# mandt-lab/shallow-ntc

Measured on AMD Instinct MI355X. Metric: decode Mpixels/s + (bpp, PSNR) on Kodak, two_layer_syn, higher is better.
Workload: dtype f32

## Files before the change

include/sntc.h:

```cpp
#ifndef SNTC_H_
#define SNTC_H_

#include <stddef.h>
#include <stdint.h>

#ifdef __cplusplus
extern "C" {
#endif

#define SNTC_VERSION 100

enum {
  SNTC_OK = 0,
  SNTC_ERR_BAD_SHAPE = 1,
  SNTC_ERR_UNSUPPORTED = 2,
  SNTC_ERR_HIP = 3,
  SNTC_ERR_NONFINITE = 4,
  SNTC_ERR_NO_DEVICE = 5
};

const char* sntc_last_error(void);
int sntc_version(void);
int sntc_device_count(void);
int sntc_device_arch(int device, char* buf, size_t buflen);
// ... 113 lines not shown
int sntc_conv_launch_order(const sntc_conv_plan* plan, int n, int h, int w, int* column_major);
int64_t sntc_conv_tune_workspace_bytes(const sntc_conv_plan* plan, int n, int h, int w);
int sntc_conv_plan_tune(sntc_conv_plan* plan, const float* x, int n, int h, int w, float* y, const float* res,
                        const float* aux, void* workspace, size_t workspace_bytes, int reps, int* variant, int* stream_k,
                        void* stream);
int sntc_conv_plan_candidates(const sntc_conv_plan* plan, int n, int h, int w, int* variants, int* stream_k, int capacity);
int sntc_conv_plan_set_choice(sntc_conv_plan* plan, int n, int h, int w, int variant, int stream_k);
int sntc_conv_plan_clear_tuning(sntc_conv_plan* plan);
int sntc_conv_plan_drop_choice(sntc_conv_plan* plan, int n, int h, int w, int ncols);

int sntc_conv_columns_supported(const sntc_conv_plan* plan, int ncols);
int sntc_conv_forward_columns(const sntc_conv_plan* plan, const float* x, int n, int h, int w, float* y, const float* res,
                              const float* aux, void* workspace, size_t workspace_bytes, void* stream, int ncols);
int64_t sntc_conv_columns_flops(const sntc_conv_plan* plan, int n, int h, int w, int ncols);
int64_t sntc_conv_columns_workspace_bytes(const sntc_conv_plan* plan, int n, int h, int w, int ncols);
int sntc_conv_columns_launch_info(const sntc_conv_plan* plan, int n, int h, int w, int ncols, int* variant, int* nblocks,
                                  int* column_major);
int64_t sntc_conv_columns_tune_workspace_bytes(const sntc_conv_plan* plan, int n, int h, int w, int ncols);
int sntc_conv_columns_tune(sntc_conv_plan* plan, const float* x, int n, int h, int w, int ncols, float* y, void* workspace,
                           size_t workspace_bytes, int reps, int* variant, int* stream_k, void* stream);
int sntc_conv_columns_candidates(const sntc_conv_plan* plan, int n, int h, int w, int ncols, int* variants, int* stream_k,
                                 int capacity);
int sntc_conv_columns_set_choice(sntc_conv_plan* plan, int n, int h, int w, int ncols, int variant, int stream_k);

int sntc_gdn_small(const float* x, int64_t npix, int c, const float* beta, const float* gamma,
                   int inverse, int alpha, int epsilon_is_half, float* y, void* stream);

int sntc_two_layer_tail(const float* t, int n, int hh, int wh, int ch, int has_res, int act_kind,
                        const float* beta, const float* gamma, const float* w2, const float* b2,
                        int k2, int s2, int cout, float* x_hat, void* stream);
int sntc_two_layer_tail_pixels(const float* t, int n, int hh, int wh, int ch, int has_res, int act_kind,
                               const float* beta, const float* gamma, const float* w2, const float* b2, int k2, int s2,
                               int cout, int h, int w, const float* ref, uint8_t* pixels, uint64_t* sse, void* stream);

int sntc_pad_reflect(const float* x, int n, int h, int w, int c, int hp, int wp, float* y, void* stream);
int sntc_pad_zero(const float* x, int n, int h, int w, int c, int top, int left, int hp, int wp, float* y, void* stream);
int sntc_crop(const float* x, int n, int hp, int wp, int c, int h, int w, float* y, void* stream);
int sntc_depth_to_space(const float* x, int n, int h, int w, int c, int block, float* y, void* stream);
int sntc_concat_channels(const float* a, int ca, const float* b, int cb, int64_t npix, float* y, void* stream);
int sntc_pixels_sse(const float* x, const float* x_hat, int n, int h, int w, int c, int hs, int ws,
                    uint8_t* pixels_out, unsigned long long* sse_out, void* stream);
int sntc_block_sse(const float* x, const uint8_t* pixels, int n, int h, int w, int c, int block, uint32_t* out, void* stream);
int sntc_float_sse(const float* x, const float* x_hat, int n, int h, int w, int c, int hs, int ws,
                   double* sse_out, void* stream);

typedef struct sntc_prior sntc_prior;
int sntc_prior_create(int channels, int nlayers, const int* widths, const float* matrices,
                      const float* biases, const float* factors, void* stream, sntc_prior** prior);
void sntc_prior_destroy(sntc_prior* prior);

int sntc_entropy_factorized(const sntc_prior* prior, const float* z, int n, int64_t hw, float* z_hat,
                            double* bits, int values_only, void* stream);

int sntc_entropy_scale_normal(const float* y, const float* hyper, int n, int64_t hw, int c,
                              float* y_hat, int32_t* symbols, double* bits, int values_only,
                              void* stream);
int sntc_dequant_scale_normal(const int32_t* symbols, const float* hyper, int n, int64_t hw, int c,
                              float* y_hat, void* stream);
int sntc_dequant_mean(const int32_t* symbols, const float* mu, int n, int64_t hw, int c, int mu_stride, float* y_hat,
                      void* stream);

int64_t sntc_rans_cap_words(int64_t elems_per_image, int segments);
int sntc_rans_encode(const int32_t* values, const uint16_t* table_ids, int nimages, int64_t elems_per_image, int segments,
                     int lanes, const uint16_t* cdf, const uint32_t* meta, int ntables, int total_entries, int64_t cap_words,
                     uint16_t* scratch, int32_t* len_words, void* stream);
int sntc_rans_compact(const uint16_t* scratch, int64_t cap_words, const int32_t* len_words, const int64_t* offsets,
// ... 133 lines not shown
```

shallow-ntc_amd/_capi.py:

```python
from __future__ import annotations

import ctypes as C
import os
from pathlib import Path

_PKG = Path(__file__).resolve().parent
LIB_PATH = Path(os.environ.get("SNTC_LIB", _PKG / "lib" / "libsntc_hip.so"))

OK, ERR_BAD_SHAPE, ERR_UNSUPPORTED, ERR_HIP, ERR_NONFINITE, ERR_NO_DEVICE = range(6)

CONV2D, CONV2D_TRANSPOSE, SIGNAL_DOWN, SIGNAL_UP = range(4)
ACT_NONE, ACT_RELU, ACT_LEAKY_RELU, ACT_SIGMOID = range(4)
PRO_NONE, PRO_ABS, PRO_SQUARE = range(3)
EPI_STORE, EPI_ADD, EPI_GATE, EPI_RES_DIV, EPI_RES_MUL, EPI_RES_DIV_SQRT, EPI_RES_MUL_SQRT, EPI_MASK_RELU, EPI_MASK_LEAKY = range(9)


class SntcError(RuntimeError):
    def __init__(self, code, msg):
        super().__init__(f"sntc error {code}: {msg}")
        self.code = code


class NonFiniteError(SntcError, ValueError):
    """Mirrors tf.debugging.check_numerics' InvalidArgumentError (reference mshyper/models.py:308-309,356)."""
# ... 126 lines not shown
                                        _P, _P, _P]),
    "sntc_step_map_symbols": (C.c_int, [_P, _P, C.c_int, C.c_int64, C.c_int, C.c_int, _P, _P, _P, _P, _P, _P]),
    "sntc_step_map_table_ids": (C.c_int, [_P, C.c_int, C.c_int64, C.c_int, _P, _P, _P]),
    "sntc_dequant_step_map": (C.c_int, [_P, _P, C.c_int, C.c_int64, C.c_int, C.c_int, _P, _P, _P, _P]),
    "sntc_step_map_ladder_cost": (C.c_int, [_P, _P, C.c_int, C.c_int64, C.c_int, C.c_int, _P, _P, _P, _P, C.c_int, _P, C.c_int,
                                            C.c_int, _P, _P, _P]),
    "sntc_step_ladder_dequant": (C.c_int, [_P, _P, C.c_int, C.c_int64, C.c_int, C.c_int, _P, _P, C.c_int, _P, _P]),
    "sntc_step_map_ladder_dequant": (C.c_int, [_P, _P, C.c_int, C.c_int64, C.c_int, C.c_int, _P, _P, _P, C.c_int, _P, _P]),
    "sntc_ssim_scale": (C.c_int, [_P, _P, C.c_int, C.c_int, C.c_int, C.c_int, C.c_float, _P, _P, _P]),
    "sntc_avgpool2_symmetric": (C.c_int, [_P, C.c_int, C.c_int, C.c_int, C.c_int, _P, _P]),
    "sntc_pixels_float": (C.c_int, [_P, C.c_int, C.c_int, C.c_int, C.c_int, C.c_int, C.c_int, _P, _P]),
    "sntc_msssim_inputs": (C.c_int, [_P, _P, C.c_int, C.c_int, C.c_int, C.c_int, C.c_int, C.c_int, _P, _P, _P, _P]),
    "sntc_msssim_finish": (C.c_int, [_P, C.POINTER(C.c_double), C.POINTER(C.c_double), C.c_int, C.c_int, C.c_int, C.c_double,
                                     _P, _P, _P]),
    "sntc_ssim_scale_grad": (C.c_int, [_P, _P, C.c_int, C.c_int, C.c_int, C.c_int, C.c_float, _P, C.c_int, _P, C.c_int, C.c_int,
                                       C.c_float, _P, _P]),
    "sntc_avgpool2_symmetric_grad": (C.c_int, [_P, C.c_int, C.c_int, C.c_int, C.c_int, _P, _P]),
    "sntc_sga_factorized_fwd": (C.c_int, [_P, _P, C.c_int, C.c_int64, C.c_float, _P, C.c_uint64, C.c_uint64, _P, _P, _P, _P, _P]),
    "sntc_sga_normal_fwd": (C.c_int, [_P, _P, C.c_int, C.c_int64, C.c_int, C.c_float, _P, C.c_uint64, C.c_uint64, _P, _P, _P,
                                      _P, _P, _P]),
    "sntc_sga_normal_bwd": (C.c_int, [_P, _P, _P, _P, C.c_float, C.c_int64, C.c_int, _P, _P, _P]),
    "sntc_sga_normal_step_fwd": (C.c_int, [_P, _P, C.c_int, C.c_int64, C.c_int, C.c_float, _P, C.c_uint64, C.c_uint64, _P, _P, _P,
                                           _P, _P, _P, _P, _P, _P]),
    "sntc_sga_normal_step_bwd": (C.c_int, [_P, _P, _P, _P, C.c_float, C.c_int, C.c_int64, C.c_int, _P, _P, _P, _P, _P, _P]),
    "sntc_uq_sample": (C.c_int, [_P, _P, C.c_int64, C.c_int, C.c_int, C.c_int, C.c_float, _P, C.c_uint64, C.c_uint64, _P, _P]),
    "sntc_sga_chain": (C.c_int, [_P, _P, _P, C.c_float, C.c_int64, _P, _P]),
    "sntc_sga_normal_step_map_fwd": (C.c_int, [_P, _P, C.c_int, C.c_int64, C.c_int, C.c_float, _P, C.c_uint64, C.c_uint64, _P, _P, _P,
                                               _P, _P, _P, _P, _P]),
    "sntc_sga_normal_step_map_bwd": (C.c_int, [_P, _P, _P, _P, C.c_float, C.c_int, C.c_int64, C.c_int, _P, _P, _P, _P, _P]),
    "sntc_distortion_grad_weighted": (C.c_int, [_P, _P, C.c_int, C.c_int, C.c_int, C.c_int, C.c_int, C.c_int, C.c_float, _P, C.c_int,
                                                C.c_int, C.c_int, _P, _P, _P, _P]),
    "sntc_block_sse": (C.c_int, [_P, _P, C.c_int, C.c_int, C.c_int, C.c_int, C.c_int, _P, _P]),
    "sntc_distortion_grad": (C.c_int, [_P, _P, C.c_int, C.c_int, C.c_int, C.c_int, C.c_int, C.c_int, C.c_float, _P, _P, _P]),
    "sntc_two_layer_tail_bwd": (C.c_int, [_P, _P, C.c_int64, C.c_int, C.c_int, C.c_int, _P, _P, C.c_int, _P, _P, _P, _P]),
    "sntc_two_layer_out_adjoint": (C.c_int, [_P, C.c_int, C.c_int, C.c_int, C.c_int, _P, C.c_int, C.c_int, C.c_int, _P, _P]),
    "sntc_adam_step": (C.c_int, [_P, _P, _P, _P, C.c_int64, C.c_float, C.c_float, C.c_float, C.c_float, C.c_int64, C.c_float, _P]),
    "sntc_conv_wgrad_workspace_bytes": (C.c_int64, [C.c_int] * 9),
    "sntc_conv_wgrad": (C.c_int, [C.c_int] * 6 + [_P, _P, C.c_int, C.c_int, C.c_int, _P, C.c_int, _P, C.c_int64, _P]),
    "sntc_bias_grad_workspace_bytes": (C.c_int64, [C.c_int64, C.c_int]),
    "sntc_bias_grad": (C.c_int, [_P, C.c_int64, C.c_int, _P, C.c_int, _P, C.c_int64, _P]),
    "sntc_act_backward": (C.c_int, [_P, _P, C.c_int64, C.c_int, _P, _P]),
    "sntc_gate_forward": (C.c_int, [_P, _P, _P, C.c_int64, _P, _P]),
    "sntc_gate_backward": (C.c_int, [_P, _P, _P, C.c_int64, _P, _P, _P]),
    "sntc_axpy": (C.c_int, [_P, _P, C.c_float, C.c_int64, _P]),
    "sntc_noise_add": (C.c_int, [_P, C.c_int64, _P, C.c_uint64, C.c_uint64, _P, _P]),
    "sntc_sumsq": (C.c_int, [_P, C.c_int64, _P, _P]),
    "sntc_two_layer_hidden": (C.c_int, [_P, C.c_int64, C.c_int, C.c_int, C.c_int, _P, _P, _P, _P]),
    "sntc_gdn_reparam_forward": (C.c_int, [_P, C.c_int64, C.c_float, C.c_float, _P, _P]),
    "sntc_gdn_reparam_backward": (C.c_int, [_P, _P, C.c_int64, C.c_float, _P, _P]),
    "sntc_noisy_normal": (C.c_int, [_P, _P, C.c_int, C.c_int64, C.c_int, _P, _P, _P, _P]),
    "sntc_noisy_factorized": (C.c_int, [_P, _P, C.c_int, C.c_int64, _P, _P, _P, _P]),
    "sntc_gdn_apply": (C.c_int, [_P, _P, C.c_int64, C.c_int, _P, _P]),
    "sntc_gdn_backward_prep": (C.c_int, [_P, _P, _P, C.c_int64, C.c_int, _P, _P, _P]),
    "sntc_gdn_backward_finish": (C.c_int, [_P, _P, _P, _P, C.c_int64, C.c_int, _P, _P]),
    "sntc_small_matmul": (C.c_int, [_P, _P, C.c_int, C.c_int, C.c_int64, C.c_int, _P, _P]),
    "sntc_transpose_last2": (C.c_int, [_P, C.c_int, C.c_int, C.c_int, _P, _P]),
    "sntc_prior_record_floats": (C.c_int, [_P]),
    "sntc_prior_update": (C.c_int, [_P, _P, _P, _P, _P]),
    "sntc_prior_param_grad": (C.c_int, [_P, _P, _P, _P, C.c_float, _P, _P, _P, _P]),
}

_lib = None


def load():
    global _lib
# ... 46 lines not shown
```

shallow-ntc_amd/csrc/pixel.hip:

```cpp
#include <algorithm>
#include "sntc_internal.h"

namespace sntc {

typedef float f32x4 __attribute__((ext_vector_type(4)));

__global__ void pad_reflect_kernel(const float* __restrict__ x, int h, int w, int c, int hp, int wp,
                                   float* __restrict__ y, int64_t total) {
  for (int64_t i = blockIdx.x * (int64_t)blockDim.x + threadIdx.x; i < total; i += (int64_t)gridDim.x * blockDim.x) {
    const int k = (int)(i % c);
    int64_t t = i / c;
    const int j = (int)(t % wp);
    t /= wp;
    const int r = (int)(t % hp);
    const int64_t b = t / hp;
    const int sr = r < h ? r : 2 * h - 2 - r;
    const int sj = j < w ? j : 2 * w - 2 - j;
    y[i] = x[((b * h + sr) * w + sj) * c + k];
  }
}

__global__ void __launch_bounds__(256) pad_zero_kernel(const float* __restrict__ x, int h, int w, int c, int top, int left, int hp, int wp,
                                                       float* __restrict__ y) {
  const int64_t row = blockIdx.y;
  const int64_t b = row / hp;
  const int r = (int)(row - b * hp) - top;
  const bool row_ok = (unsigned)r < (unsigned)h;
  const int lo = left * c, hi = (left + w) * c, len = wp * c;
  const float* src = x + ((b * h + (row_ok ? r : 0)) * (int64_t)w) * c - lo;
  float* dst = y + row * (int64_t)len;
  for (int j = blockIdx.x * blockDim.x + threadIdx.x; j < len; j += gridDim.x * blockDim.x)
    dst[j] = (row_ok && j >= lo && j < hi) ? src[j] : 0.0f;
}

__global__ void crop_kernel(const float* __restrict__ x, int hp, int wp, int c, int h, int w, float* __restrict__ y,
                            int64_t total) {
  for (int64_t i = blockIdx.x * (int64_t)blockDim.x + threadIdx.x; i < total; i += (int64_t)gridDim.x * blockDim.x) {
    const int k = (int)(i % c);
// ... 125 lines not shown
  for (int i = threadIdx.x; i < C * C; i += blockDim.x) sg[i] = gamma[i];
  for (int i = threadIdx.x; i < C; i += blockDim.x) sb[i] = beta[i];
  __syncthreads();
  for (int64_t p = blockIdx.x * (int64_t)blockDim.x + threadIdx.x; p < npix; p += (int64_t)gridDim.x * blockDim.x) {
    float v[C], pool[C];
#pragma unroll
    for (int i = 0; i < C; i += 4) {
      const f32x4 t = *reinterpret_cast<const f32x4*>(x + p * C + i);
      v[i] = t[0]; v[i + 1] = t[1]; v[i + 2] = t[2]; v[i + 3] = t[3];
    }
#pragma unroll
    for (int i = 0; i < C; ++i) pool[i] = alpha == 1 ? fabsf(v[i]) : v[i] * v[i];
#pragma unroll
    for (int j0 = 0; j0 < C; j0 += 4) {
      f32x4 o;
#pragma unroll
      for (int e = 0; e < 4; ++e) {
        const int j = j0 + e;
        float nrm = sb[j];
#pragma unroll
        for (int i = 0; i < C; ++i) nrm += pool[i] * sg[i * C + j];
        if (eps_half) nrm = sqrtf(nrm);
        o[e] = inverse ? v[j] * nrm : v[j] / nrm;
      }
      *reinterpret_cast<f32x4*>(y + p * C + j0) = o;
    }
  }
}

constexpr int tail_px(int ch) { return (ch / 4) % 2 ? ch : ch + 4; }
constexpr int tail_row(int ch) { return (18 * tail_px(ch) + 63) / 64 * 64; }

template <int CH>
__global__ void __launch_bounds__(256) two_layer_tail_kernel(const float* __restrict__ t, int hh, int wh, int has_res,
                                                             int act_kind, const float* __restrict__ beta,
                                                             const float* __restrict__ gamma, const float* __restrict__ w2,
                                                             const float* __restrict__ b2, float* __restrict__ xhat,
                                                             int oh, int ow, const float* __restrict__ ref,
                                                             uint8_t* __restrict__ pix, unsigned long long* __restrict__ sse) {
  constexpr int TQ = 16, TH = TQ + 2;
  constexpr int PX = tail_px(CH), ROW = tail_row(CH);
  extern __shared__ __attribute__((aligned(16))) char smem[];
  float* sh = reinterpret_cast<float*>(smem);
  float* sg = sh + TH * ROW;
  float* sb = sg + CH * CH;
  const int img = blockIdx.z;
  const int qy0 = blockIdx.y * TQ, qx0 = blockIdx.x * TQ;
  const int c2 = has_res ? 2 * CH : CH;
  const bool use_gdn = act_kind == 1 || act_kind == 2;
  if (use_gdn) {
    for (int i = threadIdx.x; i < CH * CH; i += 256) sg[i] = gamma[i];
    for (int i = threadIdx.x; i < CH; i += 256) sb[i] = beta[i];
  }
  __syncthreads();
  for (int p = threadIdx.x; p < TH * TH; p += 256) {
    const int ly = p / TH, lx = p - ly * TH;
    const int iy = qy0 - 2 + ly, ix = qx0 - 2 + lx;
    float* dst = sh + ly * ROW + lx * PX;
    if ((unsigned)iy < (unsigned)hh && (unsigned)ix < (unsigned)wh) {
      const float* src = t + (((int64_t)img * hh + iy) * wh + ix) * c2;
      float v[CH];
#pragma unroll
      for (int i = 0; i < CH; i += 4) {
        const f32x4 q = *reinterpret_cast<const f32x4*>(src + i);
        v[i] = q[0]; v[i + 1] = q[1]; v[i + 2] = q[2]; v[i + 3] = q[3];
      }
#pragma unroll
      for (int j0 = 0; j0 < CH; j0 += 4) {
        f32x4 o;
#pragma unroll
        for (int e = 0; e < 4; ++e) {
          const int j = j0 + e;
          float r = v[j];
          if (use_gdn) {
            float nrm = sb[j];
#pragma unroll
            for (int i = 0; i < CH; ++i) nrm += fabsf(v[i]) * sg[i * CH + j];
            r = act_kind == 1 ? v[j] * nrm : v[j] / nrm;
          } else if (act_kind == 3) {
            r = fmaxf(r, 0.0f);
          } else if (act_kind == 4) {
            r = r >= 0.0f ? r : 0.2f * r;
          }
          o[e] = r;
        }
        if (has_res) {
          const f32x4 q = *reinterpret_cast<const f32x4*>(src + CH + j0);
          o = o + q;
        }
        *reinterpret_cast<f32x4*>(dst + j0) = o;
      }
    } else {
#pragma unroll
      for (int i = 0; i < CH; i += 4) *reinterpret_cast<f32x4*>(dst + i) = f32x4{0.f, 0.f, 0.f, 0.f};
    }
  }
  __syncthreads();
  const int ty = threadIdx.x >> 4, tx = threadIdx.x & 15;
  const int qy = qy0 + ty, qx = qx0 + tx;
  const int ho = 2 * hh, wo = 2 * wh;
  const float bias0 = b2[0], bias1 = b2[1], bias2 = b2[2];
  unsigned long long se = 0;
#pragma unroll
  for (int py = 0; py < 2; ++py) {
#pragma unroll
    for (int px = 0; px < 2; ++px) {
      const int oy = 2 * qy + py - 1, ox = 2 * qx + px - 1;
      float a0 = bias0, a1 = bias1, a2 = bias2;
#pragma unroll
      for (int jy = 0; jy < 3 - py; ++jy) {
#pragma unroll
        for (int jx = 0; jx < 3 - px; ++jx) {
          const int ky = py + 2 * jy, kx = px + 2 * jx;
          const float* hp = sh + (ty + 2 - jy) * ROW + (tx + 2 - jx) * PX;
          const float* wp = w2 + (ky * 5 + kx) * 3 * CH;
#pragma unroll
          for (int i = 0; i < CH; i += 4) {
            const f32x4 hv = *reinterpret_cast<const f32x4*>(hp + i);
            const f32x4 w0 = *reinterpret_cast<const f32x4*>(wp + i);
            const f32x4 w1 = *reinterpret_cast<const f32x4*>(wp + CH + i);
            const f32x4 w2v = *reinterpret_cast<const f32x4*>(wp + 2 * CH + i);
#pragma unroll
            for (int e = 0; e < 4; ++e) {
              a0 = fmaf(hv[e], w0[e], a0);
              a1 = fmaf(hv[e], w1[e], a1);
              a2 = fmaf(hv[e], w2v[e], a2);
            }
          }
        }
      }
      if (xhat && (unsigned)oy < (unsigned)ho && (unsigned)ox < (unsigned)wo) {
        float* dst = xhat + (((int64_t)img * ho + oy) * wo + ox) * 3;
        dst[0] = a0; dst[1] = a1; dst[2] = a2;
      }
      if (pix && (unsigned)oy < (unsigned)oh && (unsigned)ox < (unsigned)ow) {
        const int64_t o = (((int64_t)img * oh + oy) * ow + ox) * 3;
        const int q0 = to_pixel(a0), q1 = to_pixel(a1), q2 = to_pixel(a2);
        pix[o] = (uint8_t)q0; pix[o + 1] = (uint8_t)q1; pix[o + 2] = (uint8_t)q2;
        if (ref) {
          const int d0 = to_pixel(ref[o]) - q0, d1 = to_pixel(ref[o + 1]) - q1, d2 = to_pixel(ref[o + 2]) - q2;
          se += (unsigned)(d0 * d0 + d1 * d1 + d2 * d2);
        }
      }
    }
  }
  if (pix && ref) {
#pragma unroll
    for (int o = 32; o > 0; o >>= 1) se += __shfl_down(se, o, 64);
    unsigned long long* part = reinterpret_cast<unsigned long long*>(sg);
    __syncthreads();
    if ((threadIdx.x & 63) == 0) part[threadIdx.x >> 6] = se;
    __syncthreads();
    if (threadIdx.x == 0) atomicAdd(sse + img, part[0] + part[1] + part[2] + part[3]);
  }
}

}

using namespace sntc;

static int blocks_for(int64_t total) {
  int64_t b = (total + 255) / 256;
  return (int)(b < 1 ? 1 : (b > 2048 ? 2048 : b));
}

extern "C" int sntc_pad_reflect(const float* x, int n, int h, int w, int c, int hp, int wp, float* y, void* stream) {
  if (!x || !y) return fail(SNTC_ERR_BAD_SHAPE, "sntc_pad_reflect: null argument");
  if (n < 1 || h < 1 || w < 1 || c < 1 || hp < h || wp < w || hp - h >= h || wp - w >= w)
    return fail(SNTC_ERR_BAD_SHAPE, "sntc_pad_reflect: reflect padding needs pad < size");
  const int64_t total = (int64_t)n * hp * wp * c;
  hipLaunchKernelGGL(pad_reflect_kernel, dim3(blocks_for(total)), dim3(256), 0, (hipStream_t)stream, x, h, w, c, hp, wp, y, total);
  SNTC_HIP(hipGetLastError());
  return SNTC_OK;
}

extern "C" int sntc_pad_zero(const float* x, int n, int h, int w, int c, int top, int left, int hp, int wp, float* y, void* stream) {
  if (!x || !y) return fail(SNTC_ERR_BAD_SHAPE, "sntc_pad_zero: null argument");
  if (n < 1 || h < 1 || w < 1 || c < 1 || top < 0 || left < 0 || hp < h + top || wp < w + left)
    return fail(SNTC_ERR_BAD_SHAPE, "sntc_pad_zero: bad sizes");
  if ((int64_t)n * hp > 0x7fffffffLL / 1 || (int64_t)wp * c > 0x7fffffffLL) return fail(SNTC_ERR_BAD_SHAPE, "sntc_pad_zero: tensor too large");
  const int bx = std::max(1, std::min(8, (wp * c + 1023) / 1024));
  hipLaunchKernelGGL(pad_zero_kernel, dim3(bx, (unsigned)(n * hp)), dim3(256), 0, (hipStream_t)stream, x, h, w, c, top, left, hp, wp, y);
  SNTC_HIP(hipGetLastError());
  return SNTC_OK;
}

extern "C" int sntc_crop(const float* x, int n, int hp, int wp, int c, int h, int w, float* y, void* stream) {
// ... 101 lines not shown
  int b = blocks_for(per);
  if (b > 512) b = 512;
  hipLaunchKernelGGL(float_sse_kernel, dim3(b, n), dim3(256), 0, s, x, x_hat, h, w, c, hs, ws, sse_out);
  SNTC_HIP(hipGetLastError());
  return SNTC_OK;
}

template <int C>
static int launch_gdn(const float* x, int64_t npix, const float* beta, const float* gamma, int inverse, int alpha,
                      int eps_half, float* y, hipStream_t s) {
  hipLaunchKernelGGL((gdn_small_kernel<C>), dim3(blocks_for(npix)), dim3(256), 0, s, x, npix, beta, gamma, inverse, alpha,
                     eps_half, y);
  SNTC_HIP(hipGetLastError());
  return SNTC_OK;
}

extern "C" int sntc_gdn_small(const float* x, int64_t npix, int c, const float* beta, const float* gamma, int inverse,
                              int alpha, int epsilon_is_half, float* y, void* stream) {
  if (!x || !beta || !gamma || !y || npix < 1) return fail(SNTC_ERR_BAD_SHAPE, "sntc_gdn_small: null argument");
  if (alpha != 1 && alpha != 2) return fail(SNTC_ERR_UNSUPPORTED, "sntc_gdn_small: alpha must be 1 or 2");
  hipStream_t s = (hipStream_t)stream;
  switch (c) {
    case 4: return launch_gdn<4>(x, npix, beta, gamma, inverse, alpha, epsilon_is_half, y, s);
    case 8: return launch_gdn<8>(x, npix, beta, gamma, inverse, alpha, epsilon_is_half, y, s);
    case 12: return launch_gdn<12>(x, npix, beta, gamma, inverse, alpha, epsilon_is_half, y, s);
    case 16: return launch_gdn<16>(x, npix, beta, gamma, inverse, alpha, epsilon_is_half, y, s);
    case 24: return launch_gdn<24>(x, npix, beta, gamma, inverse, alpha, epsilon_is_half, y, s);
    case 32: return launch_gdn<32>(x, npix, beta, gamma, inverse, alpha, epsilon_is_half, y, s);
    case 48: return launch_gdn<48>(x, npix, beta, gamma, inverse, alpha, epsilon_is_half, y, s);
    default: return fail(SNTC_ERR_UNSUPPORTED, "sntc_gdn_small: channels must be one of 4,8,12,16,24,32,48");
  }
}

template <int CH>
static int launch_tail(const float* t, int n, int hh, int wh, int has_res, int act_kind, const float* beta,
                       const float* gamma, const float* w2, const float* b2, float* x_hat, int oh, int ow, const float* ref,
                       uint8_t* px, unsigned long long* sse, hipStream_t s) {
  const size_t lds = sizeof(float) * (18 * tail_row(CH) + CH * CH + CH);
  static thread_local int attr_dev = -1;
  int dev = 0;
  SNTC_HIP(hipGetDevice(&dev));
  if (attr_dev != dev) {
    SNTC_HIP(hipFuncSetAttribute(reinterpret_cast<const void*>(&two_layer_tail_kernel<CH>),
                                 hipFuncAttributeMaxDynamicSharedMemorySize, (int)lds));
    attr_dev = dev;
  }
  dim3 grid((wh + 1 + 15) / 16, (hh + 1 + 15) / 16, n);
  if (px && ref && sse) if (int zrc = zero_async(sse, sizeof(unsigned long long) * n, s)) return zrc;
  hipLaunchKernelGGL((two_layer_tail_kernel<CH>), grid, dim3(256), lds, s, t, hh, wh, has_res, act_kind, beta, gamma, w2,
                     b2, x_hat, oh, ow, ref, px, sse);
  SNTC_HIP(hipGetLastError());
  return SNTC_OK;
}

static int tail_dispatch(const float* t, int n, int hh, int wh, int ch, int has_res, int act_kind, const float* beta,
                         const float* gamma, const float* w2, const float* b2, int k2, int s2, int cout, float* x_hat, int oh,
                         int ow, const float* ref, uint8_t* px, unsigned long long* sse, void* stream) {
  if (!t || !w2 || !b2 || (!x_hat && !px)) return fail(SNTC_ERR_BAD_SHAPE, "sntc_two_layer_tail: null argument");
  if (n < 1 || hh < 1 || wh < 1) return fail(SNTC_ERR_BAD_SHAPE, "sntc_two_layer_tail: empty input");
  if (k2 != 5 || s2 != 2 || cout != 3)
    return fail(SNTC_ERR_UNSUPPORTED, "sntc_two_layer_tail: only the 5x5 / stride-2 / 3-channel output layer is fused");
  if (act_kind < 0 || act_kind > 4) return fail(SNTC_ERR_UNSUPPORTED, "sntc_two_layer_tail: unknown activation");
  if ((act_kind == 1 || act_kind == 2) && (!beta || !gamma))
    return fail(SNTC_ERR_BAD_SHAPE, "sntc_two_layer_tail: GDN parameters missing");
  if (n > 65535) return fail(SNTC_ERR_BAD_SHAPE, "sntc_two_layer_tail: batch too large");
  if (px && (oh < 1 || ow < 1 || oh > 2 * hh || ow > 2 * wh))
    return fail(SNTC_ERR_BAD_SHAPE, "sntc_two_layer_tail_pixels: crop must lie inside the reconstruction");
  if (ref && !sse) return fail(SNTC_ERR_BAD_SHAPE, "sntc_two_layer_tail_pixels: a reference needs an sse output");
  hipStream_t s = (hipStream_t)stream;
  switch (ch) {
    case 12: return launch_tail<12>(t, n, hh, wh, has_res, act_kind, beta, gamma, w2, b2, x_hat, oh, ow, ref, px, sse, s);
    case 24: return launch_tail<24>(t, n, hh, wh, has_res, act_kind, beta, gamma, w2, b2, x_hat, oh, ow, ref, px, sse, s);
    case 48: return launch_tail<48>(t, n, hh, wh, has_res, act_kind, beta, gamma, w2, b2, x_hat, oh, ow, ref, px, sse, s);
    default: return fail(SNTC_ERR_UNSUPPORTED, "sntc_two_layer_tail: hidden channels must be 12, 24 or 48");
  }
}

extern "C" int sntc_two_layer_tail(const float* t, int n, int hh, int wh, int ch, int has_res, int act_kind,
                                   const float* beta, const float* gamma, const float* w2, const float* b2, int k2,
                                   int s2, int cout, float* x_hat, void* stream) {
  if (!x_hat) return fail(SNTC_ERR_BAD_SHAPE, "sntc_two_layer_tail: null argument");
  return tail_dispatch(t, n, hh, wh, ch, has_res, act_kind, beta, gamma, w2, b2, k2, s2, cout, x_hat, 0, 0, nullptr, nullptr,
                       nullptr, stream);
}

extern "C" int sntc_two_layer_tail_pixels(const float* t, int n, int hh, int wh, int ch, int has_res, int act_kind,
                                          const float* beta, const float* gamma, const float* w2, const float* b2, int k2,
                                          int s2, int cout, int h, int w, const float* ref, uint8_t* pixels, uint64_t* sse,
                                          void* stream) {
  if (!pixels) return fail(SNTC_ERR_BAD_SHAPE, "sntc_two_layer_tail_pixels: null argument");
  return tail_dispatch(t, n, hh, wh, ch, has_res, act_kind, beta, gamma, w2, b2, k2, s2, cout, nullptr, h, w, ref, pixels,
                       reinterpret_cast<unsigned long long*>(sse), stream);
}
```

shallow-ntc_amd/ops.py:

```python
from __future__ import annotations

import ctypes as C
import os

import numpy as np
import torch

from . import _capi as capi

ACTS = {None: capi.ACT_NONE, "none": capi.ACT_NONE, "relu": capi.ACT_RELU, "leaky_relu": capi.ACT_LEAKY_RELU,
        "lrelu": capi.ACT_LEAKY_RELU, "sigmoid": capi.ACT_SIGMOID}
KINDS = {"conv": capi.CONV2D, "convT": capi.CONV2D_TRANSPOSE, "sigdown": capi.SIGNAL_DOWN, "sigup": capi.SIGNAL_UP}


WGRAD_STREAM = None
FUSE_RESIDUAL_TAIL = True
MEAN_ONLY_HYPER = True
FUSE_RESIDUAL_BLOCK = not os.environ.get("SNTC_NO_RB_FUSE")
FUSED_BLOCK_MIN_TILES = 256
CONCURRENT_BRANCHES = not os.environ.get("SNTC_NO_BRANCH_STREAMS")
CONCURRENT_BRANCH_MAX_TILES = 1024
MAX_INPUT_BYTES = 1 << 31
PROFILE = None
ROW_PACKED_FIRST_LAYER = not os.environ.get("SNTC_NO_ROWPACK")
# ... 706 lines not shown


class static_schedules:

    def __init__(self, active=True):
        self.active = bool(active)

    def __enter__(self):
        self._was = stream_k_enabled()
        if self.active and self._was:
            set_stream_k(False)
        return self

    def __exit__(self, *exc):
        if self.active and self._was:
            set_stream_k(True)
        return False


def gdn_small(x, beta, gamma, inverse=False, alpha=1, epsilon=1.0):
    _check_nhwc(x)
    c = x.shape[-1]
    y = torch.empty_like(x)
    capi.call("sntc_gdn_small", _ptr(x), x.numel() // c, c, _ptr(beta), _ptr(gamma), int(inverse), int(alpha),
              int(epsilon == 0.5), _ptr(y), _stream())
    return y


GDN_SMALL_CHANNELS = (4, 8, 12, 16, 24, 32, 48)
TAIL_CHANNELS = (12, 24, 48)
TAIL_ACTS = {None: 0, "none": 0, "igdn": 1, "igdn1": 1, "gdn": 2, "gdn1": 2, "relu": 3, "leaky_relu": 4, "lrelu": 4}


def _tail_profile(n, hh, wh, ch, cout, k2, s2):
    prof = PROFILE
    if prof is None:
        return None
    e0, e1 = torch.cuda.Event(enable_timing=True), torch.cuda.Event(enable_timing=True)
    e0.record()
    return prof, dict(e0=e0, e1=e1, flops=2 * n * hh * wh * k2 * k2 * ch * cout, variant=0, nblocks=0, vec=True, kind="tail",
                      k=k2, s=s2, cin=ch, cout=cout, n=n, h=hh, w=wh)


def _tail_profile_done(rec):
    if rec is not None:
        rec[1]["e1"].record()
        rec[0].append(rec[1])


def two_layer_tail(t, ch, has_res, act_kind, beta, gamma, w2, b2, k2=5, s2=2):
    _check_nhwc(t, ch * (2 if has_res else 1))
    n, hh, wh, _ = t.shape
    cout = int(w2.shape[2])
    y = torch.empty((n, hh * s2, wh * s2, cout), dtype=torch.float32, device=t.device)
    rec = _tail_profile(n, hh, wh, ch, cout, k2, s2)
    capi.call("sntc_two_layer_tail", _ptr(t), n, hh, wh, ch, int(has_res), act_kind, _ptr(beta), _ptr(gamma),
              _ptr(w2), _ptr(b2), k2, s2, cout, _ptr(y), _stream())
    _tail_profile_done(rec)
    return y


def two_layer_tail_pixels(t, ch, has_res, act_kind, beta, gamma, w2, b2, h, w, reference=None, k2=5, s2=2):
    _check_nhwc(t, ch * (2 if has_res else 1))
    n, hh, wh, _ = t.shape
    cout = int(w2.shape[2])
    px = torch.empty((n, h, w, cout), dtype=torch.uint8, device=t.device)
    sse = None
    if reference is not None:
        _check_nhwc(reference, cout)
        if tuple(reference.shape) != (n, h, w, cout):
            raise ValueError(f"reference {tuple(reference.shape)} does not match the decoded size {(n, h, w, cout)}")
        sse = torch.empty((n,), dtype=torch.int64, device=t.device)
    rec = _tail_profile(n, hh, wh, ch, cout, k2, s2)
    capi.call("sntc_two_layer_tail_pixels", _ptr(t), n, hh, wh, ch, int(has_res), act_kind, _ptr(beta), _ptr(gamma), _ptr(w2),
              _ptr(b2), k2, s2, cout, h, w, _ptr(reference), _ptr(px), _ptr(sse), _stream())
    _tail_profile_done(rec)
    return px, sse


def pad_zero(x, top, left, bottom, right):
    _check_nhwc(x)
    n, h, w, c = x.shape
    y = torch.empty((n, h + top + bottom, w + left + right, c), dtype=torch.float32, device=x.device)
    capi.call("sntc_pad_zero", _ptr(x), n, h, w, c, top, left, h + top + bottom, w + left + right, _ptr(y), _stream())
    return y


class RowPackedConv:

    def __init__(self, weight, bias, stride, act=None):
        self.k, self.stride = int(weight.shape[0]), int(stride)
        self.plan = ConvPlan("conv", weight, bias, stride, act, rowpack=True)
        self.cin, self.cout = self.plan.cin, self.plan.cout

    def _pads(self, size):
        out = -(-size // self.stride)
        total = max((out - 1) * self.stride + self.k - size, 0)
        return total // 2, total - total // 2

    def out_hw(self, h, w):
        return -(-h // self.stride), -(-w // self.stride)

    def flops(self, n, h, w):
        ho, wo = self.out_hw(h, w)
        return 2 * n * ho * wo * self.k * self.k * self.cin * self.cout
# ... 840 lines not shown
```

Measured before the change: 3940.

## Add phase-aligned tail kernel with packed weights and staged pixel stores

Adds a new two-layer tail kernel where each thread computes a 2x2 block of output pixels from a 3x3 neighbourhood of hidden pixels (polyphase transposed conv), using a 1-pixel halo instead of 2. It uses weights repacked into paired float2 layout for vector FMA, and stages uint8 pixels in LDS for coalesced 16-byte stores. A small pack kernel runs on every call to reorder w2 into a cached per-stream buffer. The new path is enabled by default with a runtime switch, at the cost of an extra launch per call and more LDS.

Result: no change. 3932 (-0.2%).

```diff
diff --git a/include/sntc.h b/include/sntc.h
--- a/include/sntc.h
+++ b/include/sntc.h
@@ -169,6 +169,7 @@
 int sntc_two_layer_tail_pixels(const float* t, int n, int hh, int wh, int ch, int has_res, int act_kind,
                                const float* beta, const float* gamma, const float* w2, const float* b2, int k2, int s2,
                                int cout, int h, int w, const float* ref, uint8_t* pixels, uint64_t* sse, void* stream);
+int sntc_tail_set_aligned(int enabled);
 
 int sntc_pad_reflect(const float* x, int n, int h, int w, int c, int hp, int wp, float* y, void* stream);
 int sntc_pad_zero(const float* x, int n, int h, int w, int c, int top, int left, int hp, int wp, float* y, void* stream);
diff --git a/shallow-ntc_amd/_capi.py b/shallow-ntc_amd/_capi.py
--- a/shallow-ntc_amd/_capi.py
+++ b/shallow-ntc_amd/_capi.py
@@ -182,6 +182,7 @@
                                                 C.c_int, C.c_int, _P, _P, _P, _P]),
     "sntc_block_sse": (C.c_int, [_P, _P, C.c_int, C.c_int, C.c_int, C.c_int, C.c_int, _P, _P]),
     "sntc_distortion_grad": (C.c_int, [_P, _P, C.c_int, C.c_int, C.c_int, C.c_int, C.c_int, C.c_int, C.c_float, _P, _P, _P]),
+    "sntc_tail_set_aligned": (C.c_int, [C.c_int]),
     "sntc_two_layer_tail_bwd": (C.c_int, [_P, _P, C.c_int64, C.c_int, C.c_int, C.c_int, _P, _P, C.c_int, _P, _P, _P, _P]),
     "sntc_two_layer_out_adjoint": (C.c_int, [_P, C.c_int, C.c_int, C.c_int, C.c_int, _P, C.c_int, C.c_int, C.c_int, _P, _P]),
     "sntc_adam_step": (C.c_int, [_P, _P, _P, _P, C.c_int64, C.c_float, C.c_float, C.c_float, C.c_float, C.c_int64, C.c_float, _P]),
diff --git a/shallow-ntc_amd/csrc/pixel.hip b/shallow-ntc_amd/csrc/pixel.hip
--- a/shallow-ntc_amd/csrc/pixel.hip
+++ b/shallow-ntc_amd/csrc/pixel.hip
@@ -1,9 +1,14 @@
 #include <algorithm>
+#include <atomic>
+#include <map>
+#include <mutex>
+#include <utility>
 #include "sntc_internal.h"
 
 namespace sntc {
 
 typedef float f32x4 __attribute__((ext_vector_type(4)));
+typedef float f32x2 __attribute__((ext_vector_type(2)));
 
 __global__ void pad_reflect_kernel(const float* __restrict__ x, int h, int w, int c, int hp, int wp,
                                    float* __restrict__ y, int64_t total) {
@@ -195,30 +200,15 @@
 constexpr int tail_row(int ch) { return (18 * tail_px(ch) + 63) / 64 * 64; }
 
 template <int CH>
-__global__ void __launch_bounds__(256) two_layer_tail_kernel(const float* __restrict__ t, int hh, int wh, int has_res,
-                                                             int act_kind, const float* __restrict__ beta,
-                                                             const float* __restrict__ gamma, const float* __restrict__ w2,
-                                                             const float* __restrict__ b2, float* __restrict__ xhat,
-                                                             int oh, int ow, const float* __restrict__ ref,
-                                                             uint8_t* __restrict__ pix, unsigned long long* __restrict__ sse) {
-  constexpr int TQ = 16, TH = TQ + 2;
-  constexpr int PX = tail_px(CH), ROW = tail_row(CH);
-  extern __shared__ __attribute__((aligned(16))) char smem[];
-  float* sh = reinterpret_cast<float*>(smem);
-  float* sg = sh + TH * ROW;
-  float* sb = sg + CH * CH;
-  const int img = blockIdx.z;
-  const int qy0 = blockIdx.y * TQ, qx0 = blockIdx.x * TQ;
+__device__ __forceinline__ void tail_stage1(const float* __restrict__ t, int img, int hh, int wh, int has_res, int act_kind, int y0,
+                                            int x0, float* __restrict__ sh, const float* __restrict__ sg,
+                                            const float* __restrict__ sb) {
+  constexpr int TH = 18, PX = tail_px(CH), ROW = tail_row(CH);
   const int c2 = has_res ? 2 * CH : CH;
   const bool use_gdn = act_kind == 1 || act_kind == 2;
-  if (use_gdn) {
-    for (int i = threadIdx.x; i < CH * CH; i += 256) sg[i] = gamma[i];
-    for (int i = threadIdx.x; i < CH; i += 256) sb[i] = beta[i];
-  }
-  __syncthreads();
   for (int p = threadIdx.x; p < TH * TH; p += 256) {
     const int ly = p / TH, lx = p - ly * TH;
-    const int iy = qy0 - 2 + ly, ix = qx0 - 2 + lx;
+    const int iy = y0 + ly, ix = x0 + lx;
     float* dst = sh + ly * ROW + lx * PX;
     if ((unsigned)iy < (unsigned)hh && (unsigned)ix < (unsigned)wh) {
       const float* src = t + (((int64_t)img * hh + iy) * wh + ix) * c2;
@@ -258,6 +248,39 @@
       for (int i = 0; i < CH; i += 4) *reinterpret_cast<f32x4*>(dst + i) = f32x4{0.f, 0.f, 0.f, 0.f};
     }
   }
+}
+
+__device__ __forceinline__ void tail_sse_reduce(unsigned long long se, unsigned long long* part, unsigned long long* __restrict__ sse) {
+#pragma unroll
+  for (int o = 32; o > 0; o >>= 1) se += __shfl_down(se, o, 64);
+  __syncthreads();
+  if ((threadIdx.x & 63) == 0) part[threadIdx.x >> 6] = se;
+  __syncthreads();
+  if (threadIdx.x == 0) atomicAdd(sse, part[0] + part[1] + part[2] + part[3]);
+}
+
+template <int CH>
+__global__ void __launch_bounds__(256) two_layer_tail_kernel(const float* __restrict__ t, int hh, int wh, int has_res,
+                                                             int act_kind, const float* __restrict__ beta,
+                                                             const float* __restrict__ gamma, const float* __restrict__ w2,
+                                                             const float* __restrict__ b2, float* __restrict__ xhat,
+                                                             int oh, int ow, const float* __restrict__ ref,
+                                                             uint8_t* __restrict__ pix, unsigned long long* __restrict__ sse) {
+  constexpr int TQ = 16, TH = TQ + 2;
+  constexpr int PX = tail_px(CH), ROW = tail_row(CH);
+  extern __shared__ __attribute__((aligned(16))) char smem[];
+  float* sh = reinterpret_cast<float*>(smem);
+  float* sg = sh + TH * ROW;
+  float* sb = sg + CH * CH;
+  const int img = blockIdx.z;
+  const int qy0 = blockIdx.y * TQ, qx0 = blockIdx.x * TQ;
+  const bool use_gdn = act_kind == 1 || act_kind == 2;
+  if (use_gdn) {
+    for (int i = threadIdx.x; i < CH * CH; i += 256) sg[i] = gamma[i];
+    for (int i = threadIdx.x; i < CH; i += 256) sb[i] = beta[i];
+  }
+  __syncthreads();
+  tail_stage1<CH>(t, img, hh, wh, has_res, act_kind, qy0 - 2, qx0 - 2, sh, sg, sb);
   __syncthreads();
   const int ty = threadIdx.x >> 4, tx = threadIdx.x & 15;
   const int qy = qy0 + ty, qx = qx0 + tx;
@@ -307,15 +330,123 @@
       }
     }
   }
-  if (pix && ref) {
-#pragma unroll
-    for (int o = 32; o > 0; o >>= 1) se += __shfl_down(se, o, 64);
-    unsigned long long* part = reinterpret_cast<unsigned long long*>(sg);
-    __syncthreads();
-    if ((threadIdx.x & 63) == 0) part[threadIdx.x >> 6] = se;
-    __syncthreads();
-    if (threadIdx.x == 0) atomicAdd(sse + img, part[0] + part[1] + part[2] + part[3]);
-  }
+  if (pix && ref) tail_sse_reduce(se, reinterpret_cast<unsigned long long*>(sg), sse + img);
+}
+
+constexpr int tail_pack_floats(int ch) { return 75 * ch; }
+__host__ __device__ constexpr int tail_pack_pair(int ch, int ky, int p, int c) { return ky * 15 * ch + (p * 3 + c) * ch * 2; }
+__host__ __device__ constexpr int tail_pack_single(int ch, int ky, int c) { return ky * 15 * ch + 12 * ch + c * ch; }
+
+__global__ void __launch_bounds__(256) tail_pack_kernel(const float* __restrict__ w2, int ch, float* __restrict__ wpk) {
+  for (int s = threadIdx.x; s < 75 * ch; s += 256) {
+    const int i = s % ch, c = (s / ch) % 3, kx = (s / (3 * ch)) % 5, ky = s / (15 * ch);
+    const int d = kx == 0 ? tail_pack_single(ch, ky, c) + i : tail_pack_pair(ch, ky, (kx - 1) >> 1, c) + 2 * i + ((kx - 1) & 1);
+    wpk[d] = w2[s];
+  }
+}
+
+template <int CH>
+__global__ void __launch_bounds__(256) two_layer_tail_aligned_kernel(const float* __restrict__ t, int hh, int wh, int has_res,
+                                                                     int act_kind, const float* __restrict__ beta,
+                                                                     const float* __restrict__ gamma, const float* __restrict__ wpk,
+                                                                     const float* __restrict__ b2, float* __restrict__ xhat,
+                                                                     int oh, int ow, const float* __restrict__ ref,
+                                                                     uint8_t* __restrict__ pix, unsigned long long* __restrict__ sse) {
+  constexpr int TQ = 16, TH = TQ + 2, PX = tail_px(CH), ROW = tail_row(CH);
+  constexpr int PROW = 2 * TQ * 3;
+  extern __shared__ __attribute__((aligned(16))) char smem[];
+  float* sh = reinterpret_cast<float*>(smem);
+  float* sg = sh + TH * ROW;
+  float* sb = sg + CH * CH;
+  uint8_t* spx = reinterpret_cast<uint8_t*>(sb + CH);
+  const int img = blockIdx.z;
+  const int qy0 = blockIdx.y * TQ, qx0 = blockIdx.x * TQ;
+  if (act_kind == 1 || act_kind == 2) {
+    for (int i = threadIdx.x; i < CH * CH; i += 256) sg[i] = gamma[i];
+    for (int i = threadIdx.x; i < CH; i += 256) sb[i] = beta[i];
+  }
+  __syncthreads();
+  tail_stage1<CH>(t, img, hh, wh, has_res, act_kind, qy0 - 1, qx0 - 1, sh, sg, sb);
+  __syncthreads();
+  const int ty = threadIdx.x >> 4, tx = threadIdx.x & 15;
+  f32x2 acc[2][3];
+#pragma unroll
+  for (int c = 0; c < 3; ++c) acc[0][c] = acc[1][c] = f32x2{b2[c], b2[c]};
+#pragma unroll
+  for (int dy = 1; dy >= -1; --dy) {
+#pragma unroll
+    for (int dx = 1; dx >= -1; --dx) {
+      const float* hp = sh + (ty + 1 + dy) * ROW + (tx + 1 + dx) * PX;
+#pragma unroll
+      for (int i = 0; i < CH; i += 4) {
+        const f32x4 hv = *reinterpret_cast<const f32x4*>(hp + i);
+#pragma unroll
+        for (int e = 0; e < 4; ++e) {
+#pragma unroll
+          for (int ry = 0; ry < 2; ++ry) {
+            if (ry == 0 && dy == 1) continue;
+            const int ky = 1 - ry + 2 * (ry - dy);
+#pragma unroll
+            for (int c = 0; c < 3; ++c) {
+              if (dx == 1) {
+                acc[ry][c][1] = fmaf(hv[e], wpk[tail_pack_single(CH, ky, c) + i + e], acc[ry][c][1]);
+              } else {
+                const f32x2 w = *reinterpret_cast<const f32x2*>(wpk + tail_pack_pair(CH, ky, -dx, c) + 2 * (i + e));
+                acc[ry][c] = __builtin_elementwise_fma(f32x2{hv[e], hv[e]}, w, acc[ry][c]);
+              }
+            }
+          }
+        }
+      }
+    }
+  }
+  const int y0 = 2 * qy0, x0 = 2 * qx0;
+  if (xhat && qy0 + ty < hh && qx0 + tx < wh) {
+    const int wo = 2 * wh;
+#pragma unroll
+    for (int ry = 0; ry < 2; ++ry) {
+      float* dst = xhat + (((int64_t)img * 2 * hh + y0 + 2 * ty + ry) * wo + x0 + 2 * tx) * 3;
+#pragma unroll
+      for (int c = 0; c < 3; ++c) { dst[c] = acc[ry][c][0]; dst[3 + c] = acc[ry][c][1]; }
+    }
+  }
+  if (!pix) return;
+  unsigned long long se = 0;
+#pragma unroll
+  for (int ry = 0; ry < 2; ++ry) {
+    const int oy = y0 + 2 * ty + ry;
+    int q[6];
+#pragma unroll
+    for (int c = 0; c < 3; ++c) { q[c] = to_pixel(acc[ry][c][0]); q[3 + c] = to_pixel(acc[ry][c][1]); }
+    unsigned short* d = reinterpret_cast<unsigned short*>(spx + (2 * ty + ry) * PROW + 6 * tx);
+#pragma unroll
+    for (int k = 0; k < 3; ++k) d[k] = (unsigned short)(q[2 * k] | (q[2 * k + 1] << 8));
+    if (ref && oy < oh) {
+#pragma unroll
+      for (int rx = 0; rx < 2; ++rx) {
+        const int ox = x0 + 2 * tx + rx;
+        if (ox < ow) {
+          const int64_t o = (((int64_t)img * oh + oy) * ow + ox) * 3;
+          const int d0 = to_pixel(ref[o]) - q[3 * rx], d1 = to_pixel(ref[o + 1]) - q[3 * rx + 1], d2 = to_pixel(ref[o + 2]) - q[3 * rx + 2];
+          se += (unsigned)(d0 * d0 + d1 * d1 + d2 * d2);
+        }
+      }
+    }
+  }
+  __syncthreads();
+  const int rows = min(2 * TQ, oh - y0), rowb = min(PROW, (ow - x0) * 3);
+  const int r = threadIdx.x / (PROW / 16), v = threadIdx.x - r * (PROW / 16);
+  if (r < rows && v * 16 < rowb) {
+    uint8_t* dst = pix + (((int64_t)img * oh + y0 + r) * ow + x0) * 3 + v * 16;
+    const uint8_t* src = spx + r * PROW + v * 16;
+    if (v * 16 + 16 <= rowb && (reinterpret_cast<uintptr_t>(dst) & 15) == 0) {
+      *reinterpret_cast<uint4*>(dst) = *reinterpret_cast<const uint4*>(src);
+    } else {
+      const int nb = min(16, rowb - v * 16);
+      for (int k = 0; k < nb; ++k) dst[k] = src[k];
+    }
+  }
+  if (ref) tail_sse_reduce(se, reinterpret_cast<unsigned long long*>(sg), sse + img);
 }
 
 }
@@ -483,21 +614,52 @@
   }
 }
 
+static std::atomic<int> g_tail_aligned{1};
+
+static int tail_pack_buffer(int dev, hipStream_t s, float** out) {
+  static std::mutex mu;
+  static std::map<std::pair<int, hipStream_t>, float*> bufs;
+  std::lock_guard<std::mutex> lock(mu);
+  float*& p = bufs[std::make_pair(dev, s)];
+  if (!p) {
+    hipStreamCaptureMode mode = hipStreamCaptureModeRelaxed;
+    SNTC_HIP(hipThreadExchangeStreamCaptureMode(&mode));
+    const hipError_t e = hipMalloc(&p, sizeof(float) * tail_pack_floats(48));
+    SNTC_HIP(hipThreadExchangeStreamCaptureMode(&mode));
+    if (e != hipSuccess) { p = nullptr; return hip_fail(e, "hipMalloc(tail weights)"); }
+  }
+  *out = p;
+  return SNTC_OK;
+}
+
 template <int CH>
 static int launch_tail(const float* t, int n, int hh, int wh, int has_res, int act_kind, const float* beta,
                        const float* gamma, const float* w2, const float* b2, float* x_hat, int oh, int ow, const float* ref,
                        uint8_t* px, unsigned long long* sse, hipStream_t s) {
-  const size_t lds = sizeof(float) * (18 * tail_row(CH) + CH * CH + CH);
+  const size_t lds = sizeof(float) * (18 * tail_row(CH) + CH * CH + CH), lds_aligned = lds + 32 * 32 * 3;
   static thread_local int attr_dev = -1;
   int dev = 0;
   SNTC_HIP(hipGetDevice(&dev));
   if (attr_dev != dev) {
     SNTC_HIP(hipFuncSetAttribute(reinterpret_cast<const void*>(&two_layer_tail_kernel<CH>),
                                  hipFuncAttributeMaxDynamicSharedMemorySize, (int)lds));
+    SNTC_HIP(hipFuncSetAttribute(reinterpret_cast<const void*>(&two_layer_tail_aligned_kernel<CH>),
+                                 hipFuncAttributeMaxDynamicSharedMemorySize, (int)lds_aligned));
     attr_dev = dev;
   }
+  if (px && ref && sse) if (int zrc = zero_async(sse, sizeof(unsigned long long) * n, s)) return zrc;
+  if (g_tail_aligned.load(std::memory_order_relaxed)) {
+    float* wpk = nullptr;
+    if (int rc = tail_pack_buffer(dev, s, &wpk)) return rc;
+    hipLaunchKernelGGL(tail_pack_kernel, dim3(1), dim3(256), 0, s, w2, CH, wpk);
+    SNTC_HIP(hipGetLastError());
+    const int qh = x_hat ? hh : (oh + 1) / 2, qw = x_hat ? wh : (ow + 1) / 2;
+    hipLaunchKernelGGL((two_layer_tail_aligned_kernel<CH>), dim3((qw + 15) / 16, (qh + 15) / 16, n), dim3(256), lds_aligned, s, t, hh,
+                       wh, has_res, act_kind, beta, gamma, wpk, b2, x_hat, oh, ow, ref, px, sse);
+    SNTC_HIP(hipGetLastError());
+    return SNTC_OK;
+  }
   dim3 grid((wh + 1 + 15) / 16, (hh + 1 + 15) / 16, n);
-  if (px && ref && sse) if (int zrc = zero_async(sse, sizeof(unsigned long long) * n, s)) return zrc;
   hipLaunchKernelGGL((two_layer_tail_kernel<CH>), grid, dim3(256), lds, s, t, hh, wh, has_res, act_kind, beta, gamma, w2,
                      b2, x_hat, oh, ow, ref, px, sse);
   SNTC_HIP(hipGetLastError());
@@ -543,3 +705,8 @@
   return tail_dispatch(t, n, hh, wh, ch, has_res, act_kind, beta, gamma, w2, b2, k2, s2, cout, nullptr, h, w, ref, pixels,
                        reinterpret_cast<unsigned long long*>(sse), stream);
 }
+
+extern "C" int sntc_tail_set_aligned(int enabled) {
+  g_tail_aligned.store(enabled ? 1 : 0, std::memory_order_relaxed);
+  return SNTC_OK;
+}
diff --git a/shallow-ntc_amd/ops.py b/shallow-ntc_amd/ops.py
--- a/shallow-ntc_amd/ops.py
+++ b/shallow-ntc_amd/ops.py
@@ -762,6 +762,18 @@
 TAIL_ACTS = {None: 0, "none": 0, "igdn": 1, "igdn1": 1, "gdn": 2, "gdn1": 2, "relu": 3, "leaky_relu": 4, "lrelu": 4}
 
 
+TAIL_ALIGNED = True
+_tail_aligned_set = None
+
+
+def _sync_tail_switch():
+    global _tail_aligned_set
+    want = bool(TAIL_ALIGNED)
+    if want != _tail_aligned_set:
+        capi.call("sntc_tail_set_aligned", int(want))
+        _tail_aligned_set = want
+
+
 def _tail_profile(n, hh, wh, ch, cout, k2, s2):
     prof = PROFILE
     if prof is None:
@@ -783,6 +795,7 @@
     n, hh, wh, _ = t.shape
     cout = int(w2.shape[2])
     y = torch.empty((n, hh * s2, wh * s2, cout), dtype=torch.float32, device=t.device)
+    _sync_tail_switch()
     rec = _tail_profile(n, hh, wh, ch, cout, k2, s2)
     capi.call("sntc_two_layer_tail", _ptr(t), n, hh, wh, ch, int(has_res), act_kind, _ptr(beta), _ptr(gamma),
               _ptr(w2), _ptr(b2), k2, s2, cout, _ptr(y), _stream())
@@ -801,6 +814,7 @@
         if tuple(reference.shape) != (n, h, w, cout):
             raise ValueError(f"reference {tuple(reference.shape)} does not match the decoded size {(n, h, w, cout)}")
         sse = torch.empty((n,), dtype=torch.int64, device=t.device)
+    _sync_tail_switch()
     rec = _tail_profile(n, hh, wh, ch, cout, k2, s2)
     capi.call("sntc_two_layer_tail_pixels", _ptr(t), n, hh, wh, ch, int(has_res), act_kind, _ptr(beta), _ptr(gamma), _ptr(w2),
               _ptr(b2), k2, s2, cout, h, w, _ptr(reference), _ptr(px), _ptr(sse), _stream())
```
